# skyhehe123/SA-SSD

Measured on NVIDIA H100. Metric: KITTI frames/sec (~20k pts, car_cfg voxel grid), higher is better.
Workload: dtype f32

## Files before the change

### sa-ssd_b200/csrc/conv2d_tma.cu

```cuda
#include <cuda.h>

#include <cstdlib>

#include "tc_common.cuh"

namespace tma {

using namespace tc;

constexpr int TILE_H = SASSD_CONV2D_TILE_H, TILE_W = SASSD_CONV2D_TILE_W;
constexpr int BKC = 64;
constexpr int kConstTile = 1 << 30;
constexpr int kBgTile = 1 << 29;
constexpr int CONS_WARPS = CONS_THREADS / 32;
constexpr int W_LOAD = CONS_WARPS;

constexpr int A_ROWS = TILE_H + 2;
constexpr int A_PLANE_BYTES = A_ROWS * TILE_W * 128;
constexpr int A_STAGE_BYTES = 2 * A_PLANE_BYTES;

constexpr int FRAG_BLOCK_BYTES = 128 * 32;
constexpr int OUT_PITCH = 64 + 4;

template <int BN>
struct Cfg2 {
    static constexpr bool RS = BN >= 128;
    static constexpr int THREADS = CONS_THREADS + (RS ? 128 : 32);
    static constexpr int A_STAGES = RS ? 3 : 2;
    static constexpr int B_TILE_BYTES = BN * 128;
    static constexpr int B_STAGE_BYTES = 2 * B_TILE_BYTES;
    static constexpr int B_STAGES = RS ? 0 : 6;
    static constexpr int OUT_BYTES = RS ? 2 * TILE_H * TILE_W * OUT_PITCH * 4 : 0;
    static constexpr int RING_BYTES = A_STAGES * A_STAGE_BYTES + B_STAGES * B_STAGE_BYTES + OUT_BYTES;
    static constexpr int ORDER_CAP = 4608;
    static constexpr int SMEM_BYTES = RING_BYTES + 1024 + 256 + ORDER_CAP / 4 + ORDER_CAP * 2;
    static_assert(SMEM_BYTES <= 227 * 1024, "dynamic shared memory above the sm_90 limit");
};

__device__ __forceinline__ void tma_load_4d(uint32_t dst, const CUtensorMap* map, int c0, int c1, int c2, int c3,
                                            uint32_t bar) {
    asm volatile(
        "cp.async.bulk.tensor.4d.shared::cluster.global.tile.mbarrier::complete_tx::bytes [%0], [%1, {%2, %3, %4, %5}], [%6];"
        ::"r"(dst), "l"(map), "r"(c0), "r"(c1), "r"(c2), "r"(c3), "r"(bar)
        : "memory");
}

struct Conv2dArgs {
    const void* wpack;
    const float* scale;
    const float* shift;
    float* out_f32;
    __half* out_split;
    int batch, H, W, cin, cout, taps, relu, out_f32_stride, out_split_ch;
    const int* tile_dist;
    const float* cvec;
    int reach;
    int* counters;
    int tile_order;
    int nsplit;
};

struct Background {
    const __half* split;
    const float* f32;
};

__device__ __forceinline__ int tile_skip_flag(const Conv2dArgs& p, const Background& bg, int dist, int ty, int tx,
                                              int tiles_y, int tiles_x) {
    if (dist <= p.reach) return 0;
    if (p.reach < 2 || !(ty == 0 || ty == tiles_y - 1 || tx == 0 || tx == tiles_x - 1)) return kConstTile;
    return (bg.split || bg.f32) ? kBgTile : 0;
}

__device__ __forceinline__ void copy_background_unit(const Conv2dArgs& p, const Background& bg, int b, int ty, int tx,
                                                     int n_off, int bn, int tid, int nthreads) {
    const size_t hw = (size_t)p.H * p.W;
    if (p.out_split) {
        const int vpp = min(bn, p.out_split_ch - n_off) >> 3;
        const size_t bg_plane = hw * p.out_split_ch, plane = (size_t)p.batch * bg_plane;
        for (int i = tid; i < TILE_H * TILE_W * vpp; i += nthreads) {
            const int pix = i / vpp;
            const int y = ty * TILE_H + pix / TILE_W, x = tx * TILE_W + pix % TILE_W;
            if (y >= p.H || x >= p.W) continue;
            const size_t src = ((size_t)y * p.W + x) * p.out_split_ch + n_off + 8 * (i % vpp);
            const uint4 hi = __ldg((const uint4*)(bg.split + src));
            const uint4 lo = __ldg((const uint4*)(bg.split + bg_plane + src));
            __half* dst = p.out_split + (size_t)b * bg_plane + src;
            *(uint4*)dst = hi;
            *(uint4*)(dst + plane) = lo;
        }
    }
    if (p.out_f32) {
        const int vpp = min(bn, p.out_f32_stride - n_off) >> 2;
        for (int i = tid; i < TILE_H * TILE_W * vpp; i += nthreads) {
            const int pix = i / vpp;
            const int y = ty * TILE_H + pix / TILE_W, x = tx * TILE_W + pix % TILE_W;
            if (y >= p.H || x >= p.W) continue;
            const size_t src = ((size_t)y * p.W + x) * p.out_f32_stride + n_off + 4 * (i % vpp);
            *(float4*)(p.out_f32 + (size_t)b * hw * p.out_f32_stride + src) = __ldg((const float4*)(bg.f32 + src));
        }
    }
}

template <int EW>
__device__ __forceinline__ void store_constant_unit(const Conv2dArgs& p, int b, int ty, int tx, int n_off, int ncols,
                                                    int warp, int lane) {
    const int vpp = ncols >> 3, g = lane % vpp, sub = lane / vpp, ppi = 32 / vpp;
    const int c = n_off + 8 * g;
    float v[8];
#pragma unroll
    for (int j = 0; j < 8; ++j) v[j] = (c + j) < p.cout ? __ldg(&p.cvec[c + j]) : 0.f;
    uint4 hi, lo;
    split_f16x2(v[0], v[1], hi.x, lo.x);
    split_f16x2(v[2], v[3], hi.y, lo.y);
    split_f16x2(v[4], v[5], hi.z, lo.z);
    split_f16x2(v[6], v[7], hi.w, lo.w);
    const size_t plane = (size_t)p.batch * p.H * p.W * p.out_split_ch;
#pragma unroll 4
    for (int pg = warp; pg * ppi < TILE_H * TILE_W; pg += EW) {
        const int pix = pg * ppi + sub;
        const int y = ty * TILE_H + pix / TILE_W, x = tx * TILE_W + pix % TILE_W;
        if (y < p.H && x < p.W) {
            __half* dst = p.out_split + (((size_t)b * p.H + y) * p.W + x) * p.out_split_ch + c;
            *(uint4*)dst = hi;
            *(uint4*)(dst + plane) = lo;
        }
    }
}

__device__ __forceinline__ void zero_split_tail(const Conv2dArgs& p, int b, int ty, int tx, int c0, int tid,
                                                int nthreads) {
    if (!p.out_split || c0 >= p.out_split_ch) return;
    const int vpp = (p.out_split_ch - c0) >> 3;
    const size_t plane = (size_t)p.batch * p.H * p.W * p.out_split_ch;
    const uint4 zero = make_uint4(0u, 0u, 0u, 0u);
    for (int i = tid; i < TILE_H * TILE_W * vpp; i += nthreads) {
        const int pix = i / vpp;
        const int y = ty * TILE_H + pix / TILE_W, x = tx * TILE_W + pix % TILE_W;
        if (y >= p.H || x >= p.W) continue;
        __half* dst = p.out_split + (((size_t)b * p.H + y) * p.W + x) * p.out_split_ch + c0 + 8 * (i % vpp);
        *(uint4*)dst = zero;
        *(uint4*)(dst + plane) = zero;
    }
}

__device__ __forceinline__ void mma_chunk_x3_rs(float (&big)[64], float (&small)[64], const uint32_t (&w)[32],
                                                uint32_t x_hi, uint32_t x_lo) {
    const uint64_t dxh = make_desc(x_hi), dxl = make_desc(x_lo);
#pragma unroll
    for (int k = 0; k < 4; ++k) {
        const uint64_t ko = 2ull * (uint64_t)k;
        const uint32_t wh[4] = {w[8 * k], w[8 * k + 1], w[8 * k + 2], w[8 * k + 3]};
        const uint32_t wl[4] = {w[8 * k + 4], w[8 * k + 5], w[8 * k + 6], w[8 * k + 7]};
        wgmma_rs_n128(small, wh, dxl + ko);
        wgmma_rs_n128(small, wl, dxh + ko);
        wgmma_rs_n128(big, wh, dxh + ko);
    }
}

template <int BN>
__global__ void __launch_bounds__(Cfg2<BN>::THREADS, 1)
conv2d_tma_kernel(const __grid_constant__ CUtensorMap amap, const Conv2dArgs p, const Background bg) {
    using C = Cfg2<BN>;
    constexpr int A_STAGES = C::A_STAGES;
    extern __shared__ uint8_t smem_raw[];
    __shared__ int s_ncomp;
    __shared__ int s_walk[6];
    const uint32_t base = (smem_u32(smem_raw) + 1023u) & ~1023u;
    uint8_t* base_ptr = smem_raw + (base - smem_u32(smem_raw));
    const uint32_t b_ring = base + A_STAGES * A_STAGE_BYTES;
    const uint32_t bar_base = base + C::RING_BYTES;
    auto a_full = [&](int s) { return bar_base + 8u * s; };
    auto a_empty = [&](int s) { return bar_base + 8u * (A_STAGES + s); };
    auto b_full = [&](int s) { return bar_base + 8u * (2 * A_STAGES + s); };
    auto b_empty = [&](int s) { return bar_base + 8u * (2 * A_STAGES + C::B_STAGES + s); };

    pdl_launch_dependents();
    const int warp = __shfl_sync(0xffffffffu, (int)(threadIdx.x >> 5), 0), lane = threadIdx.x & 31;
    const int tiles_x = (p.W + TILE_W - 1) / TILE_W, tiles_y = (p.H + TILE_H - 1) / TILE_H;
    const int ntiles = p.batch * tiles_y * tiles_x;
    const int nsplit = p.nsplit, nunits = ntiles * nsplit;
    const int kchunks = (p.cin + BKC - 1) / BKC;
    const int nchunks = p.taps * kchunks;
    const int ncols = p.taps == 9 ? 3 : 1, nrows = ncols, halo = ncols / 2;

    if (threadIdx.x == 0) {
        for (int s = 0; s < A_STAGES; ++s) { mbar_init(a_full(s), 1); mbar_init(a_empty(s), 2); }
        for (int s = 0; s < C::B_STAGES; ++s) { mbar_init(b_full(s), 1); mbar_init(b_empty(s), 2); }
        fence_barrier_init();
        asm volatile("prefetch.tensormap [%0];" ::"l"(&amap) : "memory");
        s_walk[0] = s_walk[1] = nunits;
        s_walk[2] = s_walk[4] = nunits + blockIdx.x;
        s_walk[3] = 1;
        s_walk[5] = blockIdx.x;
    }
    __syncthreads();
    pdl_wait();

    uint32_t* verdict = (uint32_t*)(base_ptr + C::RING_BYTES + 256);
    uint16_t* order = (uint16_t*)(verdict + 2 * (C::ORDER_CAP / 32));
    const bool small_map = p.tile_dist != nullptr && ntiles <= C::ORDER_CAP;
    const bool use_order = p.tile_order && small_map;
    if (small_map) {
        const int nslots = (ntiles + 31) / 32;
#pragma unroll 1
        for (int i0 = 4 * warp; i0 < nslots; i0 += 4 * (C::THREADS / 32)) {
            int dist[4];
#pragma unroll
            for (int e = 0; e < 4; ++e) {
                const int t = (i0 + e) * 32 + lane;
                dist[e] = t < ntiles ? __ldg(&p.tile_dist[t]) : 0;
            }
#pragma unroll
            for (int e = 0; e < 4; ++e) {
                const int t = (i0 + e) * 32 + lane;
                const int f = t < ntiles ? tile_skip_flag(p, bg, dist[e], (t / tiles_x) % tiles_y, t % tiles_x, tiles_y,
                                                          tiles_x) : 0;
                const uint32_t cst = __ballot_sync(0xffffffffu, f == kConstTile);
                const uint32_t bgm = __ballot_sync(0xffffffffu, f == kBgTile);
                if (lane == 0 && i0 + e < nslots) {
                    verdict[i0 + e] = cst;
                    verdict[C::ORDER_CAP / 32 + i0 + e] = bgm;
                }
            }
        }
        __syncthreads();
        if (warp == 0) {
            auto word = [&](int t, uint32_t cst, uint32_t bgm) {
                return (uint16_t)(t | (((cst >> lane) & 1u) ? 0x8000 : 0) | (((bgm >> lane) & 1u) ? 0x4000 : 0));
            };
            if (use_order) {
                int n = 0;
                for (int pass = 0; pass < 2; ++pass) {
#pragma unroll 1
                    for (int i = 0; i < nslots; ++i) {
                        const int t = i * 32 + lane;
                        const uint32_t cst = verdict[i], bgm = verdict[C::ORDER_CAP / 32 + i];
                        const bool skip = ((cst | bgm) >> lane) & 1u;
                        const bool take = t < ntiles && (skip == (pass == 1));
                        const uint32_t m = __ballot_sync(0xffffffffu, take);
                        if (take) order[n + __popc(m & ((1u << lane) - 1u))] = word(t, cst, bgm);
                        n += __popc(m);
                    }
                    if (pass == 0 && lane == 0) s_ncomp = n;
                }
                if (lane == 0) {
                    constexpr int kTailAbsorb = 8;
                    const int G = gridDim.x, c = blockIdx.x;
                    const int ucomp = s_ncomp * nsplit;
                    const int heavy = ucomp % G, light = G - heavy;
                    const int absorb = heavy ? min(nunits - ucomp, kTailAbsorb * light) : 0;
                    const int s2 = ucomp + c - heavy, s3 = ucomp + absorb + c;
                    const int first_tail = (c >= heavy && s2 < ucomp + absorb) ? s2 : s3;
                    s_walk[0] = ucomp;
                    s_walk[1] = ucomp + absorb;
                    s_walk[2] = first_tail;
                    s_walk[3] = light;
                    s_walk[4] = s3;
                    s_walk[5] = c < ucomp ? c : first_tail;
                }
            } else {
#pragma unroll 1
                for (int i = 0; i < nslots; ++i) {
                    const int t = i * 32 + lane;
                    if (t < ntiles) order[t] = word(t, verdict[i], verdict[C::ORDER_CAP / 32 + i]);
                }
            }
        }
        __syncthreads();
    }
    auto next_unit = [&](int k) -> int {
        if (k < s_walk[0]) { k += gridDim.x; return k < s_walk[0] ? k : s_walk[2]; }
        if (k < s_walk[1]) { k += s_walk[3]; return k < s_walk[1] ? k : s_walk[4]; }
        return k + gridDim.x;
    };
    auto tile_ref = [&](int k) -> int {
        if (small_map) { const int v = order[k]; return (v & 0x3fff) | ((v & 0xc000) << 15); }
        if (!p.tile_dist) return k;
        return k | tile_skip_flag(p, bg, __ldg(&p.tile_dist[k]), (k / tiles_x) % tiles_y, k % tiles_x, tiles_y, tiles_x);
    };

    if (warp >= W_LOAD) {
        if constexpr (C::RS) {
            setmaxnreg_dec<40>();
            if (warp != W_LOAD) return;
        }
        if (lane == 0) {
            int a_stage = 0, b_stage = 0;
            uint32_t a_phase = 0, b_phase = 0;
            const uint32_t a_bytes = 2u * (TILE_H + 2 * halo) * TILE_W * 128;
            for (int k = s_walk[5]; k < nunits; k = next_unit(k)) {
                const int ref = tile_ref(k / nsplit), half = k % nsplit;
                if (ref & (kConstTile | kBgTile)) continue;
                const int tile = ref;
                const int b = tile / (tiles_y * tiles_x);
                const int ty = (tile / tiles_x) % tiles_y, tx = tile % tiles_x;
                const int y0 = ty * TILE_H, x0 = tx * TILE_W;
                for (int col = 0; col < ncols; ++col) {
                    const int dx = col - halo;
                    for (int kc = 0; kc < kchunks; ++kc) {
                        mbar_wait(a_empty(a_stage), a_phase ^ 1u);
                        const uint32_t a_hi = base + a_stage * A_STAGE_BYTES;
                        mbar_expect_tx(a_full(a_stage), a_bytes);
                        tma_load_4d(a_hi, &amap, kc * BKC, x0 + dx, y0 - halo, b, a_full(a_stage));
                        tma_load_4d(a_hi + A_PLANE_BYTES, &amap, kc * BKC, x0 + dx, y0 - halo, p.batch + b, a_full(a_stage));
                        if (++a_stage == A_STAGES) { a_stage = 0; a_phase ^= 1u; }
                        if constexpr (!C::RS) {
                            for (int row = 0; row < nrows; ++row) {
                                const int t = row * ncols + col;
                                mbar_wait(b_empty(b_stage), b_phase ^ 1u);
                                const uint32_t b_dst = b_ring + b_stage * C::B_STAGE_BYTES;
                                mbar_expect_tx(b_full(b_stage), C::B_STAGE_BYTES);
                                const uint8_t* src = (const uint8_t*)p.wpack +
                                                     (size_t)(t * kchunks + kc) * (size_t)(2 * nsplit) * C::B_TILE_BYTES +
                                                     (size_t)half * C::B_TILE_BYTES;
                                constexpr uint32_t kPiece = (C::B_TILE_BYTES >= 8192) ? 8192u : (uint32_t)C::B_TILE_BYTES;
#pragma unroll 1
                                for (int part = 0; part < 2; ++part)
#pragma unroll 1
                                    for (uint32_t o = 0; o < (uint32_t)C::B_TILE_BYTES; o += kPiece)
                                        bulk_g2s(b_dst + part * C::B_TILE_BYTES + o,
                                                 src + (size_t)part * nsplit * C::B_TILE_BYTES + o, kPiece, b_full(b_stage));
                                if (++b_stage == C::B_STAGES) { b_stage = 0; b_phase ^= 1u; }
                            }
                        }
                    }
                }
            }
        }
        if (p.out_split && nsplit * BN < p.out_split_ch) {
            __syncwarp();
            for (int k = s_walk[5]; k < nunits; k = next_unit(k)) {
                if (k % nsplit != nsplit - 1) continue;
                const int tile = tile_ref(k / nsplit) & ~(kConstTile | kBgTile);
                zero_split_tail(p, tile / (tiles_y * tiles_x), (tile / tiles_x) % tiles_y, tile % tiles_x, nsplit * BN,
                                lane, 32);
            }
        }
    } else {
        if constexpr (C::RS) setmaxnreg_inc<232>();
        const int wg = threadIdx.x >> 7, t = threadIdx.x & 127;
        const int rl0 = wg * 64 + (t >> 5) * 16 + ((t & 31) >> 2);
        const size_t plane = (size_t)p.batch * p.H * p.W * p.out_split_ch;
        float big[BN / 2], small[BN / 2];
        int a_stage = 0, b_stage = 0;
        uint32_t a_phase = 0, b_phase = 0;
        int computed = 0;
        for (int k = s_walk[5]; k < nunits; k = next_unit(k)) {
            const int ref = tile_ref(k / nsplit), n_off = (k % nsplit) * BN;
            const int tile = ref & ~(kConstTile | kBgTile);
            const bool const_tile = (ref & kConstTile) != 0;
            const int b = tile / (tiles_y * tiles_x);
            const int ty = (tile / tiles_x) % tiles_y, tx = tile % tiles_x;
            if (ref & kBgTile) continue;
            if (const_tile) {
                const int ncols = min(BN, p.out_split_ch - n_off);
                if (p.out_split && !p.out_f32 && (ncols == 64 || ncols == 128 || ncols == 256)) {
                    store_constant_unit<CONS_WARPS>(p, b, ty, tx, n_off, ncols, warp, lane);
                    continue;
                }
            } else {
                if (k % nsplit == 0) ++computed;
#pragma unroll
                for (int i = 0; i < BN / 2; ++i) { big[i] = 0.f; small[i] = 0.f; }
                int prev_b = -1, prev_a = -1, row = 0;
                if constexpr (C::RS) {
                    const uint32_t kstep = 2u * nsplit * FRAG_BLOCK_BYTES, qstep = 4u * kstep;
                    const uint8_t* wsrc = (const uint8_t*)p.wpack + (2 * (k % nsplit) + wg) * FRAG_BLOCK_BYTES + t * 32;
                    auto load_w = [&](uint32_t (&w)[32], int q) {
                        const uint8_t* src = wsrc + (size_t)q * qstep;
#pragma unroll
                        for (int s = 0; s < 4; ++s) {
                            const uint4 h = ldg_nc_v4(src + s * kstep), l = ldg_nc_v4(src + s * kstep + 16);
                            w[8 * s] = h.x; w[8 * s + 1] = h.y; w[8 * s + 2] = h.z; w[8 * s + 3] = h.w;
                            w[8 * s + 4] = l.x; w[8 * s + 5] = l.y; w[8 * s + 6] = l.z; w[8 * s + 7] = l.w;
                        }
                    };
                    auto chunk = [&](uint32_t (&w)[32], uint32_t (&w_next)[32], int ch) {
                        if (row == 0) mbar_wait(a_full(a_stage), a_phase);
                        const uint32_t xh = base + a_stage * A_STAGE_BYTES + (uint32_t)row * (TILE_W * 128u);
                        wgmma_fence();
                        mma_chunk_x3_rs(big, small, w, xh, xh + A_PLANE_BYTES);
                        wgmma_commit();
                        wgmma_wait<1>();
                        fence_regs<32>(w_next);
                        if (t == 0 && prev_a >= 0) mbar_arrive(a_empty(prev_a));
                        if (ch + 1 < nchunks) load_w(w_next, ch + 1);
                        prev_a = -1;
                        if (++row == nrows) {
                            row = 0;
                            prev_a = a_stage;
                            if (++a_stage == A_STAGES) { a_stage = 0; a_phase ^= 1u; }
                        }
                    };
                    uint32_t wa[32], wb[32];
                    load_w(wa, 0);
                    for (int ch = 0; ch < nchunks; ch += 2) {
                        chunk(wa, wb, ch);
                        if (ch + 1 == nchunks) break;
                        chunk(wb, wa, ch + 1);
                    }
                    wgmma_wait<0>();
                    fence_regs<32>(wa);
                    fence_regs<32>(wb);
                } else {
                    for (int ch = 0; ch < nchunks; ++ch) {
                        if (row == 0) mbar_wait(a_full(a_stage), a_phase);
                        mbar_wait(b_full(b_stage), b_phase);
                        const uint32_t ah = base + a_stage * A_STAGE_BYTES + (uint32_t)(row * TILE_W + wg * 64) * 128u;
                        const uint32_t bh = b_ring + b_stage * C::B_STAGE_BYTES;
                        wgmma_fence();
                        mma_chunk_x3<1, BN>(big, small, ah, ah + A_PLANE_BYTES, bh, bh + C::B_TILE_BYTES);
                        wgmma_commit();
                        wgmma_wait<1>();
                        if (t == 0) {
                            if (prev_b >= 0) mbar_arrive(b_empty(prev_b));
                            if (prev_a >= 0) mbar_arrive(a_empty(prev_a));
                        }
                        prev_b = b_stage;
                        if (++b_stage == C::B_STAGES) { b_stage = 0; b_phase ^= 1u; }
                        prev_a = -1;
                        if (++row == nrows) {
                            row = 0;
                            prev_a = a_stage;
                            if (++a_stage == A_STAGES) { a_stage = 0; a_phase ^= 1u; }
                        }
                    }
                }
                wgmma_wait<0>();
                fence_regs<BN / 2>(big);
                fence_regs<BN / 2>(small);
                if (t == 0) {
                    if (prev_b >= 0) mbar_arrive(b_empty(prev_b));
                    if (prev_a >= 0) mbar_arrive(a_empty(prev_a));
                }
            }
            if constexpr (C::RS) {
                float* stage = (float*)(base_ptr + A_STAGES * A_STAGE_BYTES) + wg * (TILE_H * TILE_W * OUT_PITCH);
                const int m0 = 16 * (t >> 5) + ((t & 31) >> 2), c_wg = n_off + 64 * wg;
                float cv[2], sc[2], sh[2];
#pragma unroll
                for (int i = 0; i < 2; ++i) {
                    const int n = c_wg + m0 + 8 * i;
                    cv[i] = const_tile && n < p.cout ? __ldg(&p.cvec[n]) : 0.f;
                    sc[i] = p.scale && n < p.cout ? __ldg(&p.scale[n]) : 1.f;
                    sh[i] = p.shift && n < p.cout ? __ldg(&p.shift[n]) : 0.f;
                }
                named_bar_sync(1 + wg, 128);
#pragma unroll
                for (int j = 0; j < 16; ++j)
#pragma unroll
                    for (int i = 0; i < 2; ++i)
#pragma unroll
                        for (int e = 0; e < 2; ++e) {
                            float o = cv[i];
                            if (!const_tile) {
                                o = fmaf(__fadd_rn(big[4 * j + 2 * i + e], small[4 * j + 2 * i + e] * (1.f / kF16LoScale)),
                                         sc[i], sh[i]);
                                if (p.relu) o = fmaxf(o, 0.f);
                                if (c_wg + m0 + 8 * i >= p.cout) o = 0.f;
                            }
                            stage[(8 * j + 2 * (t & 3) + e) * OUT_PITCH + m0 + 8 * i] = o;
                        }
                named_bar_sync(1 + wg, 128);
                if (p.out_f32) {
                    for (int v = t; v < TILE_H * TILE_W * 16; v += 128) {
                        const int pix = v >> 4, c = 4 * (v & 15), n = c_wg + c;
                        const int y = ty * TILE_H + pix / TILE_W, x = tx * TILE_W + pix % TILE_W;
                        if (n >= p.out_f32_stride || y >= p.H || x >= p.W) continue;
                        *(float4*)(p.out_f32 + (((size_t)b * p.H + y) * p.W + x) * p.out_f32_stride + n) =
                            *(const float4*)(stage + pix * OUT_PITCH + c);
                    }
                }
                if (p.out_split) {
                    for (int v = t; v < TILE_H * TILE_W * 8; v += 128) {
                        const int pix = v >> 3, c = 8 * (v & 7), n = c_wg + c;
                        const int y = ty * TILE_H + pix / TILE_W, x = tx * TILE_W + pix % TILE_W;
                        if (n >= p.out_split_ch || y >= p.H || x >= p.W) continue;
                        const float4 f0 = *(const float4*)(stage + pix * OUT_PITCH + c);
                        const float4 f1 = *(const float4*)(stage + pix * OUT_PITCH + c + 4);
                        uint4 hi, lo;
                        split_f16x2(f0.x, f0.y, hi.x, lo.x);
                        split_f16x2(f0.z, f0.w, hi.y, lo.y);
                        split_f16x2(f1.x, f1.y, hi.z, lo.z);
                        split_f16x2(f1.z, f1.w, hi.w, lo.w);
                        __half* dst = p.out_split + (((size_t)b * p.H + y) * p.W + x) * p.out_split_ch + n;
                        *(uint4*)dst = hi;
                        *(uint4*)(dst + plane) = lo;
                    }
                }
            } else {
#pragma unroll
                for (int j = 0; j < BN / 8; ++j) {
                    const int n = n_off + 8 * j + 2 * (t & 3);
                    float c0, c1, sc0 = 1.f, sc1 = 1.f, sh0 = 0.f, sh1 = 0.f;
                    if (const_tile) {
                        c0 = n < p.cout ? __ldg(&p.cvec[n]) : 0.f;
                        c1 = n + 1 < p.cout ? __ldg(&p.cvec[n + 1]) : 0.f;
                    } else {
                        if (p.scale && n < p.cout) sc0 = __ldg(&p.scale[n]);
                        if (p.scale && n + 1 < p.cout) sc1 = __ldg(&p.scale[n + 1]);
                        if (p.shift && n < p.cout) sh0 = __ldg(&p.shift[n]);
                        if (p.shift && n + 1 < p.cout) sh1 = __ldg(&p.shift[n + 1]);
                    }
#pragma unroll
                    for (int i = 0; i < 2; ++i) {
                        const int rl = rl0 + 8 * i;
                        const int y = ty * TILE_H + rl / TILE_W, x = tx * TILE_W + rl % TILE_W;
                        float o0 = c0, o1 = c1;
                        if (!const_tile) {
                            o0 = fmaf(__fadd_rn(big[4 * j + 2 * i], small[4 * j + 2 * i] * (1.f / kF16LoScale)), sc0, sh0);
                            o1 = fmaf(__fadd_rn(big[4 * j + 2 * i + 1], small[4 * j + 2 * i + 1] * (1.f / kF16LoScale)), sc1, sh1);
                            if (p.relu) { o0 = fmaxf(o0, 0.f); o1 = fmaxf(o1, 0.f); }
                            if (n >= p.cout) o0 = 0.f;
                            if (n + 1 >= p.cout) o1 = 0.f;
                        }
                        if (y >= p.H || x >= p.W) continue;
                        const size_t pix = ((size_t)b * p.H + y) * p.W + x;
                        if (p.out_f32 && n < p.out_f32_stride)
                            *(float2*)(p.out_f32 + pix * p.out_f32_stride + n) = make_float2(o0, o1);
                        if (p.out_split && n < p.out_split_ch) {
                            uint32_t h, l;
                            split_f16x2(o0, o1, h, l);
                            __half* dst = p.out_split + pix * p.out_split_ch + n;
                            *(uint32_t*)dst = h;
                            *(uint32_t*)(dst + plane) = l;
                        }
                    }
                }
            }
        }
        if (bg.split || bg.f32) {
            for (int k = s_walk[5]; k < nunits; k = next_unit(k)) {
                const int ref = tile_ref(k / nsplit);
                if (!(ref & kBgTile)) continue;
                const int tile = ref & ~kBgTile;
                copy_background_unit(p, bg, tile / (tiles_y * tiles_x), (tile / tiles_x) % tiles_y, tile % tiles_x,
                                     (k % nsplit) * BN, BN, threadIdx.x, CONS_THREADS);
            }
        }
        if (p.counters && threadIdx.x == 0) {
            if (computed) atomicAdd(&p.counters[0], computed);
            if (blockIdx.x == 0) atomicAdd(&p.counters[1], ntiles);
        }
    }
}

typedef CUresult (*EncodeTiledFn)(CUtensorMap*, CUtensorMapDataType, cuuint32_t, void*, const cuuint64_t*,
                                  const cuuint64_t*, const cuuint32_t*, const cuuint32_t*, CUtensorMapInterleave,
                                  CUtensorMapSwizzle, CUtensorMapL2promotion, CUtensorMapFloatOOBfill);

static EncodeTiledFn get_encode() {
    static EncodeTiledFn fn = nullptr;
    static bool tried = false;
    if (!tried) {
        tried = true;
        void* p = nullptr;
        cudaDriverEntryPointQueryResult q;
        if (cudaGetDriverEntryPoint("cuTensorMapEncodeTiled", &p, cudaEnableDefault, &q) == cudaSuccess &&
            q == cudaDriverEntryPointSuccess)
            fn = (EncodeTiledFn)p;
    }
    return fn;
}

template <int BN>
static int launch2(const CUtensorMap& map, const Conv2dArgs& a, const Background& bg, cudaStream_t stream) {
    using C = Cfg2<BN>;
    auto kern = conv2d_tma_kernel<BN>;
    static bool configured = false;
    if (!configured) {
        if (cudaFuncSetAttribute(kern, cudaFuncAttributeMaxDynamicSharedMemorySize, C::SMEM_BYTES) != cudaSuccess)
            return SASSD_ERR_LAUNCH;
        configured = true;
    }
    const int units = a.batch * sassd_div_up(a.H, TILE_H) * sassd_div_up(a.W, TILE_W) * a.nsplit;
    const int grid = units < sassd_num_sms() ? units : sassd_num_sms();
    if (launch_pdl(kern, dim3(grid), dim3(C::THREADS), C::SMEM_BYTES, stream, map, a, bg) != cudaSuccess) return SASSD_ERR_LAUNCH;
    return sassd_check_launch();
}

__global__ void conv2d_pack_kernel(const float* __restrict__ w, int taps, int cin, int cout, int nblk,
                                   uint32_t* __restrict__ out) {
    const int kchunks = (cin + BKC - 1) / BKC, ncols = taps == 9 ? 3 : 1, nrows = ncols;
    const long long total = (long long)taps * kchunks * 4 * nblk * (FRAG_BLOCK_BYTES / 4);
    for (long long i = blockIdx.x * (long long)blockDim.x + threadIdx.x; i < total; i += (long long)gridDim.x * blockDim.x) {
        const int word = (int)(i % 8), t = (int)((i / 8) % 128);
        long long r = i / (FRAG_BLOCK_BYTES / 4);
        const int mb = (int)(r % nblk);
        r /= nblk;
        const int s = (int)(r % 4), q = (int)(r / 4);
        const int row = q % nrows, kc = (q / nrows) % kchunks, col = q / (nrows * kchunks);
        const int tap = row * ncols + col, a = word % 4, lane = t % 32;
        const int n = 64 * mb + 16 * (t / 32) + lane / 4 + 8 * (a & 1);
        const int k = kc * BKC + 16 * s + 2 * (lane % 4) + 8 * (a >> 1);
        float hi[2], lo[2];
#pragma unroll
        for (int e = 0; e < 2; ++e) {
            const float v = (k + e < cin && n < cout) ? w[((size_t)tap * cin + k + e) * cout + n] : 0.f;
            split_f16(v, hi[e], lo[e]);
        }
        const __half2 h = word < 4 ? __floats2half2_rn(hi[0], hi[1]) : __floats2half2_rn(lo[0], lo[1]);
        out[i] = *reinterpret_cast<const uint32_t*>(&h);
    }
}

}

extern "C" size_t sassd_conv2d_pack_bytes(int taps, int cin, int cout) {
    if (!(taps == 9 || taps == 1) || cin < 1 || cout < 1 || cout > 256) return 0;
    if (cout <= 64) return sassd_gconv_pack_bytes(taps, cin, cout, SASSD_PREC_F16X3);
    return (size_t)taps * ((cin + tma::BKC - 1) / tma::BKC) * 4 * (cout <= 128 ? 2 : 4) * tma::FRAG_BLOCK_BYTES;
}

extern "C" int sassd_conv2d_pack(const float* weight, int taps, int cin, int cout, void* packed,
                                 sassd_stream_t stream_) {
    if (!weight || !packed || sassd_conv2d_pack_bytes(taps, cin, cout) == 0) return SASSD_ERR_ARG;
    if (cout <= 64) return sassd_gconv_pack(weight, taps, cin, cout, SASSD_PREC_F16X3, packed, stream_);
    const long long words = (long long)sassd_conv2d_pack_bytes(taps, cin, cout) / 4;
    tma::conv2d_pack_kernel<<<sassd_grid(words, 256), 256, 0, (cudaStream_t)stream_>>>(
        weight, taps, cin, cout, cout <= 128 ? 2 : 4, (uint32_t*)packed);
    return sassd_check_launch();
}

extern "C" int sassd_conv2d_f16x3(const sassd_conv2d_desc* d, const void* in_split, const void* wpack,
                                  const float* scale, const float* shift, float* out_f32, void* out_split,
                                  sassd_stream_t stream_) {
    return sassd_conv2d_f16x3_occ_bg(d, in_split, wpack, scale, shift, out_f32, out_split, nullptr, 0, nullptr, nullptr,
                                     nullptr, nullptr, stream_);
}

extern "C" int sassd_conv2d_f16x3_occ(const sassd_conv2d_desc* d, const void* in_split, const void* wpack,
                                      const float* scale, const float* shift, float* out_f32, void* out_split,
                                      const int32_t* tile_dist, int reach, const float* const_out, int32_t* counters,
                                      sassd_stream_t stream_) {
    return sassd_conv2d_f16x3_occ_bg(d, in_split, wpack, scale, shift, out_f32, out_split, tile_dist, reach, const_out,
                                     nullptr, nullptr, counters, stream_);
}

extern "C" int sassd_conv2d_f16x3_occ_bg(const sassd_conv2d_desc* d, const void* in_split, const void* wpack,
                                         const float* scale, const float* shift, float* out_f32, void* out_split,
                                         const int32_t* tile_dist, int reach, const float* const_out,
                                         const void* bg_split, const float* bg_f32, int32_t* counters,
                                         sassd_stream_t stream_) {
    if (tile_dist && (!const_out || reach < 0)) return SASSD_ERR_ARG;
    if ((bg_split || bg_f32) && ((out_split && !bg_split) || (out_f32 && !bg_f32))) return SASSD_ERR_ARG;
    if (tile_dist) {
        const int last_h = d ? d->H - (d->H - 1) / SASSD_CONV2D_TILE_H * SASSD_CONV2D_TILE_H : 0;
        const int last_w = d ? d->W - (d->W - 1) / SASSD_CONV2D_TILE_W * SASSD_CONV2D_TILE_W : 0;
        const int edge = last_h < last_w ? last_h : last_w;
        if (reach > SASSD_TILE_DIST_MAX || (edge < SASSD_CONV2D_TILE_H ? edge : SASSD_CONV2D_TILE_H) < reach - 1)
            return SASSD_ERR_UNSUPPORTED;
    }
    using namespace tma;
    if (!d || !in_split || !wpack || (!out_f32 && !out_split)) return SASSD_ERR_ARG;
    if (d->batch < 1 || d->H < 1 || d->W < 1 || d->cin < 1 || d->cout < 1 || d->cout > 256) return SASSD_ERR_ARG;
    if (!(d->taps == 9 || d->taps == 1) || (d->cin_stored % 64) != 0 || d->cin_stored < d->cin) return SASSD_ERR_ARG;
    if (out_split && ((d->out_split_ch % 8) != 0 || d->out_split_ch < 32)) return SASSD_ERR_ARG;
    if (out_f32 && (d->out_f32_stride % 4) != 0) return SASSD_ERR_ARG;
    EncodeTiledFn enc = get_encode();
    if (!enc) return SASSD_ERR_UNSUPPORTED;
    CUtensorMap map;
    cuuint64_t dims[4] = {(cuuint64_t)d->cin_stored, (cuuint64_t)d->W, (cuuint64_t)d->H, (cuuint64_t)(2 * d->batch)};
    cuuint64_t strides[3] = {(cuuint64_t)d->cin_stored * 2, (cuuint64_t)d->W * d->cin_stored * 2,
                             (cuuint64_t)d->H * d->W * d->cin_stored * 2};
    cuuint32_t box[4] = {(cuuint32_t)BKC, (cuuint32_t)TILE_W, (cuuint32_t)(d->taps == 9 ? A_ROWS : TILE_H), 1u};
    cuuint32_t estr[4] = {1u, 1u, 1u, 1u};
    CUresult rc = enc(&map, CU_TENSOR_MAP_DATA_TYPE_FLOAT16, 4, const_cast<void*>(in_split), dims, strides, box, estr,
                      CU_TENSOR_MAP_INTERLEAVE_NONE, CU_TENSOR_MAP_SWIZZLE_128B, CU_TENSOR_MAP_L2_PROMOTION_L2_256B,
                      CU_TENSOR_MAP_FLOAT_OOB_FILL_NONE);
    if (rc != CUDA_SUCCESS) return SASSD_ERR_LAUNCH;
    Conv2dArgs a;
    a.wpack = wpack; a.scale = scale; a.shift = shift; a.out_f32 = out_f32; a.out_split = (__half*)out_split;
    a.batch = d->batch; a.H = d->H; a.W = d->W; a.cin = d->cin; a.cout = d->cout; a.taps = d->taps; a.relu = d->relu;
    a.out_f32_stride = d->out_f32_stride; a.out_split_ch = d->out_split_ch;
    a.tile_dist = tile_dist; a.reach = reach; a.cvec = const_out; a.counters = counters;
    a.tile_order = d->tile_order;
    a.nsplit = 1;
    const Background bg = {out_split ? (const __half*)bg_split : nullptr, out_f32 ? bg_f32 : nullptr};
    cudaStream_t stream = (cudaStream_t)stream_;
    if (d->cout <= 32) return launch2<32>(map, a, bg, stream);
    if (d->cout <= 64) return launch2<64>(map, a, bg, stream);
    if (d->cout <= 128) return launch2<128>(map, a, bg, stream);
    a.nsplit = 2;
    return launch2<128>(map, a, bg, stream);
}

__global__ void sparse_to_bev_split_kernel(const float4* __restrict__ feat, const int4* __restrict__ coors,
                                           const int* __restrict__ d_rows, int rows_cap, int C4, int D, int H, int W,
                                           size_t plane, __half* __restrict__ bev, int* __restrict__ tile_dist) {
    const int rows = min(*d_rows, rows_cap);
    const long long total = (long long)rows * C4;
    for (long long i = blockIdx.x * (long long)blockDim.x + threadIdx.x; i < total;
         i += (long long)gridDim.x * blockDim.x) {
        const int r = (int)(i / C4), q = (int)(i % C4);
        const int4 c = __ldg(&coors[r]);
        const float4 v = __ldg(&feat[i]);
        uint32_t h0, h1, l0, l1;
        tc::split_f16x2(v.x, v.y, h0, l0);
        tc::split_f16x2(v.z, v.w, h1, l1);
        __half* dst = bev + ((((size_t)c.x * H + c.z) * W + c.w) * (size_t)(D * C4) + (size_t)c.y * C4 + q) * 4;
        *(uint2*)dst = make_uint2(h0, h1);
        *(uint2*)(dst + plane) = make_uint2(l0, l1);
        if (tile_dist && q == 0) sassd_mark_conv2d_tiles(tile_dist, c.x, c.z, c.w, H, W);
    }
}

extern "C" int sassd_sparse_to_bev_split(const float* feat, const int32_t* coors, const int32_t* d_rows, int rows_cap,
                                         int C, int D, int H, int W, int batch, void* bev_split, int32_t* tile_dist,
                                         sassd_stream_t stream_) {
    if (!feat || !coors || !d_rows || !bev_split || (C & 3) || batch < 1) return SASSD_ERR_ARG;
    if (rows_cap <= 0) return SASSD_OK;
    const size_t plane = (size_t)batch * H * W * D * C;
    sparse_to_bev_split_kernel<<<sassd_grid((long long)rows_cap * (C / 4), 256), 256, 0, (cudaStream_t)stream_>>>(
        (const float4*)feat, (const int4*)coors, d_rows, rows_cap, C / 4, D, H, W, plane, (__half*)bev_split, tile_dist);
    return sassd_check_launch();
}
```

### sa-ssd_b200/csrc/tc_common.cuh

```cuda
#pragma once
#include <cuda_fp16.h>

#include "common.cuh"

#include <cstdlib>
#include <utility>

namespace tc {

constexpr int BM = 128;
constexpr int BK = 32;
constexpr int A_TILE_BYTES = BM * 128;
constexpr int CONS_THREADS = 256;

__device__ __forceinline__ uint32_t smem_u32(const void* p) { return (uint32_t)__cvta_generic_to_shared(p); }

__device__ __forceinline__ void mbar_init(uint32_t bar, uint32_t count) {
    asm volatile("mbarrier.init.shared::cta.b64 [%0], %1;" ::"r"(bar), "r"(count));
}
__device__ __forceinline__ void mbar_arrive(uint32_t bar) {
    asm volatile("mbarrier.arrive.shared::cta.b64 _, [%0];" ::"r"(bar) : "memory");
}
__device__ __forceinline__ void mbar_expect_tx(uint32_t bar, uint32_t bytes) {
    asm volatile("mbarrier.arrive.expect_tx.shared::cta.b64 _, [%0], %1;" ::"r"(bar), "r"(bytes) : "memory");
}
__device__ __forceinline__ void mbar_wait(uint32_t bar, uint32_t parity) {
    asm volatile(
        "{\n\t"
        ".reg .pred p;\n\t"
        "WAIT_LOOP:\n\t"
        "mbarrier.try_wait.parity.shared::cta.b64 p, [%0], %1;\n\t"
        "@p bra.uni WAIT_DONE;\n\t"
        "bra.uni WAIT_LOOP;\n\t"
        "WAIT_DONE:\n\t"
        "}\n" ::"r"(bar), "r"(parity) : "memory");
}
__device__ __forceinline__ void pdl_launch_dependents() { asm volatile("griddepcontrol.launch_dependents;" ::: "memory"); }
__device__ __forceinline__ void pdl_wait() { asm volatile("griddepcontrol.wait;" ::: "memory"); }

__device__ __forceinline__ void fence_proxy_async() { asm volatile("fence.proxy.async.shared::cta;" ::: "memory"); }
__device__ __forceinline__ void fence_barrier_init() { asm volatile("fence.mbarrier_init.release.cluster;" ::: "memory"); }

__device__ __forceinline__ void bulk_g2s(uint32_t dst, const void* src, uint32_t bytes, uint32_t bar) {
    asm volatile("cp.async.bulk.shared::cluster.global.mbarrier::complete_tx::bytes [%0], [%1], %2, [%3];" ::"r"(dst),
                 "l"(src), "r"(bytes), "r"(bar)
                 : "memory");
}
__device__ __forceinline__ uint32_t cluster_ctarank() {
    uint32_t r;
    asm volatile("mov.u32 %0, %%cluster_ctarank;" : "=r"(r));
    return r;
}
__device__ __forceinline__ void cluster_sync_all() {
    asm volatile("barrier.cluster.arrive.release.aligned;" ::: "memory");
    asm volatile("barrier.cluster.wait.acquire.aligned;" ::: "memory");
}

__device__ __forceinline__ uint64_t make_desc(uint32_t saddr) {
    return (uint64_t)((saddr & 0x3FFFFu) >> 4) | ((uint64_t)1 << 16) | ((uint64_t)(1024 >> 4) << 32) | ((uint64_t)1 << 62);
}

__device__ __forceinline__ void wgmma_fence() { asm volatile("wgmma.fence.sync.aligned;" ::: "memory"); }
__device__ __forceinline__ void wgmma_commit() { asm volatile("wgmma.commit_group.sync.aligned;" ::: "memory"); }
template <int N>
__device__ __forceinline__ void wgmma_wait() { asm volatile("wgmma.wait_group.sync.aligned %0;" ::"n"(N) : "memory"); }
template <int R>
__device__ __forceinline__ void fence_regs(float (&d)[R]) {
#pragma unroll
    for (int i = 0; i < R; ++i) asm volatile("" : "+f"(d[i])::"memory");
}

template <int PREC, int N>
__device__ __forceinline__ void wgmma(float (&d)[N / 2], uint64_t da, uint64_t db, uint32_t scale_d);
template <>
__device__ __forceinline__ void wgmma<1, 16>(float (&d)[8], uint64_t da, uint64_t db, uint32_t scale_d) {
    asm volatile(
        "{\n\t.reg .pred p;\n\tsetp.ne.b32 p, %10, 0;\n\t"
        "wgmma.mma_async.sync.aligned.m64n16k16.f32.f16.f16 {%0, %1, %2, %3, %4, %5, %6, %7}, %8, %9, p, 1, 1, 0, 0;\n\t}\n"
        : "+f"(d[0]), "+f"(d[1]), "+f"(d[2]), "+f"(d[3]), "+f"(d[4]), "+f"(d[5]), "+f"(d[6]), "+f"(d[7])
        : "l"(da), "l"(db), "r"(scale_d) : "memory");
}
template <>
__device__ __forceinline__ void wgmma<1, 32>(float (&d)[16], uint64_t da, uint64_t db, uint32_t scale_d) {
    asm volatile(
        "{\n\t.reg .pred p;\n\tsetp.ne.b32 p, %18, 0;\n\t"
        "wgmma.mma_async.sync.aligned.m64n32k16.f32.f16.f16 {%0, %1, %2, %3, %4, %5, %6, %7, %8, %9, %10, %11, %12, %13, %14, %15}, %16, %17, p, 1, 1, 0, 0;\n\t}\n"
        : "+f"(d[0]), "+f"(d[1]), "+f"(d[2]), "+f"(d[3]), "+f"(d[4]), "+f"(d[5]), "+f"(d[6]), "+f"(d[7]), "+f"(d[8]), "+f"(d[9]), "+f"(d[10]), "+f"(d[11]), "+f"(d[12]), "+f"(d[13]), "+f"(d[14]), "+f"(d[15])
        : "l"(da), "l"(db), "r"(scale_d) : "memory");
}
template <>
__device__ __forceinline__ void wgmma<1, 64>(float (&d)[32], uint64_t da, uint64_t db, uint32_t scale_d) {
    asm volatile(
        "{\n\t.reg .pred p;\n\tsetp.ne.b32 p, %34, 0;\n\t"
        "wgmma.mma_async.sync.aligned.m64n64k16.f32.f16.f16 {%0, %1, %2, %3, %4, %5, %6, %7, %8, %9, %10, %11, %12, %13, %14, %15, %16, %17, %18, %19, %20, %21, %22, %23, %24, %25, %26, %27, %28, %29, %30, %31}, %32, %33, p, 1, 1, 0, 0;\n\t}\n"
        : "+f"(d[0]), "+f"(d[1]), "+f"(d[2]), "+f"(d[3]), "+f"(d[4]), "+f"(d[5]), "+f"(d[6]), "+f"(d[7]), "+f"(d[8]), "+f"(d[9]), "+f"(d[10]), "+f"(d[11]), "+f"(d[12]), "+f"(d[13]), "+f"(d[14]), "+f"(d[15]), "+f"(d[16]), "+f"(d[17]), "+f"(d[18]), "+f"(d[19]), "+f"(d[20]), "+f"(d[21]), "+f"(d[22]), "+f"(d[23]), "+f"(d[24]), "+f"(d[25]), "+f"(d[26]), "+f"(d[27]), "+f"(d[28]), "+f"(d[29]), "+f"(d[30]), "+f"(d[31])
        : "l"(da), "l"(db), "r"(scale_d) : "memory");
}
template <>
__device__ __forceinline__ void wgmma<1, 128>(float (&d)[64], uint64_t da, uint64_t db, uint32_t scale_d) {
    asm volatile(
        "{\n\t.reg .pred p;\n\tsetp.ne.b32 p, %66, 0;\n\t"
        "wgmma.mma_async.sync.aligned.m64n128k16.f32.f16.f16 {%0, %1, %2, %3, %4, %5, %6, %7, %8, %9, %10, %11, %12, %13, %14, %15, %16, %17, %18, %19, %20, %21, %22, %23, %24, %25, %26, %27, %28, %29, %30, %31, %32, %33, %34, %35, %36, %37, %38, %39, %40, %41, %42, %43, %44, %45, %46, %47, %48, %49, %50, %51, %52, %53, %54, %55, %56, %57, %58, %59, %60, %61, %62, %63}, %64, %65, p, 1, 1, 0, 0;\n\t}\n"
        : "+f"(d[0]), "+f"(d[1]), "+f"(d[2]), "+f"(d[3]), "+f"(d[4]), "+f"(d[5]), "+f"(d[6]), "+f"(d[7]), "+f"(d[8]), "+f"(d[9]), "+f"(d[10]), "+f"(d[11]), "+f"(d[12]), "+f"(d[13]), "+f"(d[14]), "+f"(d[15]), "+f"(d[16]), "+f"(d[17]), "+f"(d[18]), "+f"(d[19]), "+f"(d[20]), "+f"(d[21]), "+f"(d[22]), "+f"(d[23]), "+f"(d[24]), "+f"(d[25]), "+f"(d[26]), "+f"(d[27]), "+f"(d[28]), "+f"(d[29]), "+f"(d[30]), "+f"(d[31]), "+f"(d[32]), "+f"(d[33]), "+f"(d[34]), "+f"(d[35]), "+f"(d[36]), "+f"(d[37]), "+f"(d[38]), "+f"(d[39]), "+f"(d[40]), "+f"(d[41]), "+f"(d[42]), "+f"(d[43]), "+f"(d[44]), "+f"(d[45]), "+f"(d[46]), "+f"(d[47]), "+f"(d[48]), "+f"(d[49]), "+f"(d[50]), "+f"(d[51]), "+f"(d[52]), "+f"(d[53]), "+f"(d[54]), "+f"(d[55]), "+f"(d[56]), "+f"(d[57]), "+f"(d[58]), "+f"(d[59]), "+f"(d[60]), "+f"(d[61]), "+f"(d[62]), "+f"(d[63])
        : "l"(da), "l"(db), "r"(scale_d) : "memory");
}
template <>
__device__ __forceinline__ void wgmma<0, 16>(float (&d)[8], uint64_t da, uint64_t db, uint32_t scale_d) {
    asm volatile(
        "{\n\t.reg .pred p;\n\tsetp.ne.b32 p, %10, 0;\n\t"
        "wgmma.mma_async.sync.aligned.m64n16k8.f32.tf32.tf32 {%0, %1, %2, %3, %4, %5, %6, %7}, %8, %9, p, 1, 1;\n\t}\n"
        : "+f"(d[0]), "+f"(d[1]), "+f"(d[2]), "+f"(d[3]), "+f"(d[4]), "+f"(d[5]), "+f"(d[6]), "+f"(d[7])
        : "l"(da), "l"(db), "r"(scale_d) : "memory");
}
template <>
__device__ __forceinline__ void wgmma<0, 32>(float (&d)[16], uint64_t da, uint64_t db, uint32_t scale_d) {
    asm volatile(
        "{\n\t.reg .pred p;\n\tsetp.ne.b32 p, %18, 0;\n\t"
        "wgmma.mma_async.sync.aligned.m64n32k8.f32.tf32.tf32 {%0, %1, %2, %3, %4, %5, %6, %7, %8, %9, %10, %11, %12, %13, %14, %15}, %16, %17, p, 1, 1;\n\t}\n"
        : "+f"(d[0]), "+f"(d[1]), "+f"(d[2]), "+f"(d[3]), "+f"(d[4]), "+f"(d[5]), "+f"(d[6]), "+f"(d[7]), "+f"(d[8]), "+f"(d[9]), "+f"(d[10]), "+f"(d[11]), "+f"(d[12]), "+f"(d[13]), "+f"(d[14]), "+f"(d[15])
        : "l"(da), "l"(db), "r"(scale_d) : "memory");
}
template <>
__device__ __forceinline__ void wgmma<0, 64>(float (&d)[32], uint64_t da, uint64_t db, uint32_t scale_d) {
    asm volatile(
        "{\n\t.reg .pred p;\n\tsetp.ne.b32 p, %34, 0;\n\t"
        "wgmma.mma_async.sync.aligned.m64n64k8.f32.tf32.tf32 {%0, %1, %2, %3, %4, %5, %6, %7, %8, %9, %10, %11, %12, %13, %14, %15, %16, %17, %18, %19, %20, %21, %22, %23, %24, %25, %26, %27, %28, %29, %30, %31}, %32, %33, p, 1, 1;\n\t}\n"
        : "+f"(d[0]), "+f"(d[1]), "+f"(d[2]), "+f"(d[3]), "+f"(d[4]), "+f"(d[5]), "+f"(d[6]), "+f"(d[7]), "+f"(d[8]), "+f"(d[9]), "+f"(d[10]), "+f"(d[11]), "+f"(d[12]), "+f"(d[13]), "+f"(d[14]), "+f"(d[15]), "+f"(d[16]), "+f"(d[17]), "+f"(d[18]), "+f"(d[19]), "+f"(d[20]), "+f"(d[21]), "+f"(d[22]), "+f"(d[23]), "+f"(d[24]), "+f"(d[25]), "+f"(d[26]), "+f"(d[27]), "+f"(d[28]), "+f"(d[29]), "+f"(d[30]), "+f"(d[31])
        : "l"(da), "l"(db), "r"(scale_d) : "memory");
}
template <>
__device__ __forceinline__ void wgmma<0, 128>(float (&d)[64], uint64_t da, uint64_t db, uint32_t scale_d) {
    asm volatile(
        "{\n\t.reg .pred p;\n\tsetp.ne.b32 p, %66, 0;\n\t"
        "wgmma.mma_async.sync.aligned.m64n128k8.f32.tf32.tf32 {%0, %1, %2, %3, %4, %5, %6, %7, %8, %9, %10, %11, %12, %13, %14, %15, %16, %17, %18, %19, %20, %21, %22, %23, %24, %25, %26, %27, %28, %29, %30, %31, %32, %33, %34, %35, %36, %37, %38, %39, %40, %41, %42, %43, %44, %45, %46, %47, %48, %49, %50, %51, %52, %53, %54, %55, %56, %57, %58, %59, %60, %61, %62, %63}, %64, %65, p, 1, 1;\n\t}\n"
        : "+f"(d[0]), "+f"(d[1]), "+f"(d[2]), "+f"(d[3]), "+f"(d[4]), "+f"(d[5]), "+f"(d[6]), "+f"(d[7]), "+f"(d[8]), "+f"(d[9]), "+f"(d[10]), "+f"(d[11]), "+f"(d[12]), "+f"(d[13]), "+f"(d[14]), "+f"(d[15]), "+f"(d[16]), "+f"(d[17]), "+f"(d[18]), "+f"(d[19]), "+f"(d[20]), "+f"(d[21]), "+f"(d[22]), "+f"(d[23]), "+f"(d[24]), "+f"(d[25]), "+f"(d[26]), "+f"(d[27]), "+f"(d[28]), "+f"(d[29]), "+f"(d[30]), "+f"(d[31]), "+f"(d[32]), "+f"(d[33]), "+f"(d[34]), "+f"(d[35]), "+f"(d[36]), "+f"(d[37]), "+f"(d[38]), "+f"(d[39]), "+f"(d[40]), "+f"(d[41]), "+f"(d[42]), "+f"(d[43]), "+f"(d[44]), "+f"(d[45]), "+f"(d[46]), "+f"(d[47]), "+f"(d[48]), "+f"(d[49]), "+f"(d[50]), "+f"(d[51]), "+f"(d[52]), "+f"(d[53]), "+f"(d[54]), "+f"(d[55]), "+f"(d[56]), "+f"(d[57]), "+f"(d[58]), "+f"(d[59]), "+f"(d[60]), "+f"(d[61]), "+f"(d[62]), "+f"(d[63])
        : "l"(da), "l"(db), "r"(scale_d) : "memory");
}

__device__ __forceinline__ void wgmma_rs_n128(float (&d)[64], const uint32_t (&a)[4], uint64_t db) {
    asm volatile(
        "{\n\t.reg .pred p;\n\tsetp.ne.b32 p, 1, 0;\n\t"
        "wgmma.mma_async.sync.aligned.m64n128k16.f32.f16.f16 {%0, %1, %2, %3, %4, %5, %6, %7, %8, %9, %10, %11, %12, %13, %14, %15, %16, %17, %18, %19, %20, %21, %22, %23, %24, %25, %26, %27, %28, %29, %30, %31, %32, %33, %34, %35, %36, %37, %38, %39, %40, %41, %42, %43, %44, %45, %46, %47, %48, %49, %50, %51, %52, %53, %54, %55, %56, %57, %58, %59, %60, %61, %62, %63}, {%64, %65, %66, %67}, %68, p, 1, 1, 0;\n\t}\n"
        : "+f"(d[0]), "+f"(d[1]), "+f"(d[2]), "+f"(d[3]), "+f"(d[4]), "+f"(d[5]), "+f"(d[6]), "+f"(d[7]), "+f"(d[8]), "+f"(d[9]), "+f"(d[10]), "+f"(d[11]), "+f"(d[12]), "+f"(d[13]), "+f"(d[14]), "+f"(d[15]), "+f"(d[16]), "+f"(d[17]), "+f"(d[18]), "+f"(d[19]), "+f"(d[20]), "+f"(d[21]), "+f"(d[22]), "+f"(d[23]), "+f"(d[24]), "+f"(d[25]), "+f"(d[26]), "+f"(d[27]), "+f"(d[28]), "+f"(d[29]), "+f"(d[30]), "+f"(d[31]), "+f"(d[32]), "+f"(d[33]), "+f"(d[34]), "+f"(d[35]), "+f"(d[36]), "+f"(d[37]), "+f"(d[38]), "+f"(d[39]), "+f"(d[40]), "+f"(d[41]), "+f"(d[42]), "+f"(d[43]), "+f"(d[44]), "+f"(d[45]), "+f"(d[46]), "+f"(d[47]), "+f"(d[48]), "+f"(d[49]), "+f"(d[50]), "+f"(d[51]), "+f"(d[52]), "+f"(d[53]), "+f"(d[54]), "+f"(d[55]), "+f"(d[56]), "+f"(d[57]), "+f"(d[58]), "+f"(d[59]), "+f"(d[60]), "+f"(d[61]), "+f"(d[62]), "+f"(d[63])
        : "r"(a[0]), "r"(a[1]), "r"(a[2]), "r"(a[3]), "l"(db) : "memory");
}
template <int R>
__device__ __forceinline__ void fence_regs(uint32_t (&r)[R]) {
#pragma unroll
    for (int i = 0; i < R; ++i) asm volatile("" : "+r"(r[i])::"memory");
}
template <int N>
__device__ __forceinline__ void setmaxnreg_dec() { asm volatile("setmaxnreg.dec.sync.aligned.u32 %0;" ::"n"(N)); }
template <int N>
__device__ __forceinline__ void setmaxnreg_inc() { asm volatile("setmaxnreg.inc.sync.aligned.u32 %0;" ::"n"(N)); }
__device__ __forceinline__ void named_bar_sync(int id, int nthreads) {
    asm volatile("bar.sync %0, %1;" ::"r"(id), "r"(nthreads) : "memory");
}
__device__ __forceinline__ uint4 ldg_nc_v4(const void* p) {
    uint4 v;
    asm volatile("ld.global.nc.v4.u32 {%0, %1, %2, %3}, [%4];" : "=r"(v.x), "=r"(v.y), "=r"(v.z), "=r"(v.w) : "l"(p));
    return v;
}

template <int PREC, int N>
__device__ __forceinline__ void mma_chunk_x3(float (&big)[N / 2], float (&small)[N / 2], uint32_t a_hi, uint32_t a_lo,
                                             uint32_t b_hi, uint32_t b_lo, bool big_fresh = false) {
    const uint64_t dah = make_desc(a_hi), dal = make_desc(a_lo), dbh = make_desc(b_hi), dbl = make_desc(b_lo);
#pragma unroll
    for (int k = 0; k < 4; ++k) {
        const uint64_t ko = 2ull * (uint64_t)k;
        wgmma<PREC, N>(small, dal + ko, dbh + ko, 1u);
        wgmma<PREC, N>(small, dah + ko, dbl + ko, 1u);
        wgmma<PREC, N>(big, dah + ko, dbh + ko, (k == 0 && big_fresh) ? 0u : 1u);
    }
}

__device__ __forceinline__ float tf32_rn(float x) {
    uint32_t r;
    asm("cvt.rna.tf32.f32 %0, %1;" : "=r"(r) : "f"(x));
    return __uint_as_float(r);
}
__device__ __forceinline__ void split_tf32(float x, float& hi, float& lo) {
    hi = tf32_rn(x);
    lo = tf32_rn(x - hi);
}

constexpr float kF16LoScale = 2048.f;
template <int PREC>
struct Prec {
    static constexpr int BKC = PREC == 0 ? 32 : 64;
    static constexpr int NF4 = BKC / 4;
};

__device__ __forceinline__ uint32_t pack_half2(float a, float b) {
    const __half2 h = __floats2half2_rn(a, b);
    return *reinterpret_cast<const uint32_t*>(&h);
}
__device__ __forceinline__ void split_f16(float x, float& hi_as_float, float& lo_scaled) {
    const __half h = __float2half_rn(x);
    hi_as_float = __half2float(h);
    lo_scaled = (x - hi_as_float) * kF16LoScale;
}

__device__ __forceinline__ void split_f16x2(float x, float y, uint32_t& hi2, uint32_t& lo2) {
    const __half2 h = __floats2half2_rn(x, y);
    const float2 hf = __half22float2(h);
    const __half2 l = __floats2half2_rn((x - hf.x) * kF16LoScale, (y - hf.y) * kF16LoScale);
    hi2 = *reinterpret_cast<const uint32_t*>(&h);
    lo2 = *reinterpret_cast<const uint32_t*>(&l);
}

extern int g_sassd_pdl;
inline bool pdl_enabled() {
    if (g_sassd_pdl >= 0) return g_sassd_pdl != 0;
    static const bool on = [] { const char* e = getenv("SASSD_PDL"); return e && atoi(e) != 0; }();
    return on;
}
template <class... KArgs, class... Args>
inline cudaError_t launch_pdl(void (*kern)(KArgs...), dim3 grid, dim3 block, size_t smem, cudaStream_t stream,
                              Args&&... args) {
    cudaLaunchConfig_t cfg = {};
    cfg.gridDim = grid;
    cfg.blockDim = block;
    cfg.dynamicSmemBytes = smem;
    cfg.stream = stream;
    cudaLaunchAttribute attr[1];
    attr[0].id = cudaLaunchAttributeProgrammaticStreamSerialization;
    attr[0].val.programmaticStreamSerializationAllowed = 1;
    cfg.attrs = attr;
    cfg.numAttrs = pdl_enabled() ? 1 : 0;
    return cudaLaunchKernelEx(&cfg, kern, std::forward<Args>(args)...);
}

}
```

Before: 870.2.

## Stage RS-path weight fragments through a bulk-copy shared-memory ring

In the register-sourced wgmma path, weights were loaded by each consumer thread directly from global memory with non-coherent vector loads. A second producer warp now bulk-copies each chunk's weight fragments into a two-stage shared-memory ring using mbarriers, and consumers read them with shared loads, using a bank-swizzled read order, before releasing the stage. This is meant to take global load latency off the MMA critical path. In exchange the A-operand ring drops from three stages to two to free shared memory, and a named barrier per weight load is added.

```diff
diff --git a/sa-ssd_b200/csrc/conv2d_tma.cu b/sa-ssd_b200/csrc/conv2d_tma.cu
--- a/sa-ssd_b200/csrc/conv2d_tma.cu
+++ b/sa-ssd_b200/csrc/conv2d_tma.cu
@@ -26,10 +26,11 @@
 struct Cfg2 {
     static constexpr bool RS = BN >= 128;
     static constexpr int THREADS = CONS_THREADS + (RS ? 128 : 32);
-    static constexpr int A_STAGES = RS ? 3 : 2;
+    static constexpr int A_STAGES = 2;
     static constexpr int B_TILE_BYTES = BN * 128;
     static constexpr int B_STAGE_BYTES = 2 * B_TILE_BYTES;
-    static constexpr int B_STAGES = RS ? 0 : 6;
+    static_assert(!RS || B_STAGE_BYTES == 4 * 2 * FRAG_BLOCK_BYTES, "an RS weight stage holds one chunk of a unit");
+    static constexpr int B_STAGES = RS ? 2 : 6;
     static constexpr int OUT_BYTES = RS ? 2 * TILE_H * TILE_W * OUT_PITCH * 4 : 0;
     static constexpr int RING_BYTES = A_STAGES * A_STAGE_BYTES + B_STAGES * B_STAGE_BYTES + OUT_BYTES;
     static constexpr int ORDER_CAP = 4608;
@@ -283,6 +284,24 @@
     if (warp >= W_LOAD) {
         if constexpr (C::RS) {
             setmaxnreg_dec<40>();
+            if (warp == W_LOAD + 1 && lane == 0) {
+                constexpr uint32_t kStep = 2 * FRAG_BLOCK_BYTES;
+                int b_stage = 0;
+                uint32_t b_phase = 0;
+                for (int k = s_walk[5]; k < nunits; k = next_unit(k)) {
+                    if (tile_ref(k / nsplit) & (kConstTile | kBgTile)) continue;
+                    const uint8_t* src = (const uint8_t*)p.wpack + (size_t)(k % nsplit) * kStep;
+                    for (int q = 0; q < nchunks; ++q) {
+                        mbar_wait(b_empty(b_stage), b_phase ^ 1u);
+                        mbar_expect_tx(b_full(b_stage), C::B_STAGE_BYTES);
+                        const uint32_t dst = b_ring + b_stage * C::B_STAGE_BYTES;
+#pragma unroll 1
+                        for (int s = 0; s < 4; ++s, src += (size_t)nsplit * kStep)
+                            bulk_g2s(dst + s * kStep, src, kStep, b_full(b_stage));
+                        if (++b_stage == C::B_STAGES) { b_stage = 0; b_phase ^= 1u; }
+                    }
+                }
+            }
             if (warp != W_LOAD) return;
         }
         if (lane == 0) {
@@ -365,16 +384,21 @@
                 for (int i = 0; i < BN / 2; ++i) { big[i] = 0.f; small[i] = 0.f; }
                 int prev_b = -1, prev_a = -1, row = 0;
                 if constexpr (C::RS) {
-                    const uint32_t kstep = 2u * nsplit * FRAG_BLOCK_BYTES, qstep = 4u * kstep;
-                    const uint8_t* wsrc = (const uint8_t*)p.wpack + (2 * (k % nsplit) + wg) * FRAG_BLOCK_BYTES + t * 32;
-                    auto load_w = [&](uint32_t (&w)[32], int q) {
-                        const uint8_t* src = wsrc + (size_t)q * qstep;
+                    auto load_w = [&](uint32_t (&w)[32]) {
+                        mbar_wait(b_full(b_stage), b_phase);
+                        const uint32_t sw = (t & 4) * 4u;
+                        const uint32_t src = b_ring + b_stage * C::B_STAGE_BYTES + wg * FRAG_BLOCK_BYTES + t * 32;
 #pragma unroll
                         for (int s = 0; s < 4; ++s) {
-                            const uint4 h = ldg_nc_v4(src + s * kstep), l = ldg_nc_v4(src + s * kstep + 16);
+                            const uint4 x = lds_v4(src + s * 2 * FRAG_BLOCK_BYTES + sw);
+                            const uint4 y = lds_v4(src + s * 2 * FRAG_BLOCK_BYTES + (sw ^ 16u));
+                            const uint4 h = sw ? y : x, l = sw ? x : y;
                             w[8 * s] = h.x; w[8 * s + 1] = h.y; w[8 * s + 2] = h.z; w[8 * s + 3] = h.w;
                             w[8 * s + 4] = l.x; w[8 * s + 5] = l.y; w[8 * s + 6] = l.z; w[8 * s + 7] = l.w;
                         }
+                        named_bar_sync(3 + wg, 128);
+                        if (t == 0) mbar_arrive(b_empty(b_stage));
+                        if (++b_stage == C::B_STAGES) { b_stage = 0; b_phase ^= 1u; }
                     };
                     auto chunk = [&](uint32_t (&w)[32], uint32_t (&w_next)[32], int ch) {
                         if (row == 0) mbar_wait(a_full(a_stage), a_phase);
@@ -385,7 +409,7 @@
                         wgmma_wait<1>();
                         fence_regs<32>(w_next);
                         if (t == 0 && prev_a >= 0) mbar_arrive(a_empty(prev_a));
-                        if (ch + 1 < nchunks) load_w(w_next, ch + 1);
+                        if (ch + 1 < nchunks) load_w(w_next);
                         prev_a = -1;
                         if (++row == nrows) {
                             row = 0;
@@ -394,7 +418,7 @@
                         }
                     };
                     uint32_t wa[32], wb[32];
-                    load_w(wa, 0);
+                    load_w(wa);
                     for (int ch = 0; ch < nchunks; ch += 2) {
                         chunk(wa, wb, ch);
                         if (ch + 1 == nchunks) break;
@@ -436,7 +460,8 @@
                 }
             }
             if constexpr (C::RS) {
-                float* stage = (float*)(base_ptr + A_STAGES * A_STAGE_BYTES) + wg * (TILE_H * TILE_W * OUT_PITCH);
+                float* stage = (float*)(base_ptr + A_STAGES * A_STAGE_BYTES + C::B_STAGES * C::B_STAGE_BYTES) +
+                               wg * (TILE_H * TILE_W * OUT_PITCH);
                 const int m0 = 16 * (t >> 5) + ((t & 31) >> 2), c_wg = n_off + 64 * wg;
                 float cv[2], sc[2], sh[2];
 #pragma unroll
diff --git a/sa-ssd_b200/csrc/tc_common.cuh b/sa-ssd_b200/csrc/tc_common.cuh
--- a/sa-ssd_b200/csrc/tc_common.cuh
+++ b/sa-ssd_b200/csrc/tc_common.cuh
@@ -156,9 +156,10 @@
 __device__ __forceinline__ void named_bar_sync(int id, int nthreads) {
     asm volatile("bar.sync %0, %1;" ::"r"(id), "r"(nthreads) : "memory");
 }
-__device__ __forceinline__ uint4 ldg_nc_v4(const void* p) {
+__device__ __forceinline__ uint4 lds_v4(uint32_t addr) {
     uint4 v;
-    asm volatile("ld.global.nc.v4.u32 {%0, %1, %2, %3}, [%4];" : "=r"(v.x), "=r"(v.y), "=r"(v.z), "=r"(v.w) : "l"(p));
+    asm volatile("ld.shared.v4.u32 {%0, %1, %2, %3}, [%4];" : "=r"(v.x), "=r"(v.y), "=r"(v.z), "=r"(v.w) : "r"(addr)
+                 : "memory");
     return v;
 }
 
```

New measurement: 900.8 (median of 6 runs). 1.04x the previous value.
